# GRIPS-code/pyLBL

Hardware: AMD Instinct MI355X
Metric: line×gridpoint Voigt evals/sec (whole job; per GPU: evals_per_s_per_gpu; spectra/sec: spectra_per_s) (higher is better)
Workload: dtype f64; 1 GPU; BASELINE config 'target': 1 level(s) per GPU, H2O+CO2, grid 1-5000 cm-1 at 0.001 cm-1 (5000000 points), cut_off 25, remove_pedestal=False; levels_total=1, atmosphere=surface, output=gas, parallelism=levels sharded

## Files before the change

### pylbl_amd/abi.py

```python
from ctypes import CDLL, POINTER, Structure, byref, c_char_p, c_double, c_int32, c_int64, \
                   c_void_p
import os
from pathlib import Path

import numpy as np

from .errors import EngineError

LIBRARY_PATH = Path(__file__).resolve().parent / "liblbl_amd.so"

LBL_OK = 0
TABLE_OPEN_FAILED, TABLE_NO_ALIAS, TABLE_NO_TIPS, TABLE_NOT_RECTANGULAR, TABLE_NO_ISOTOPOLOGUES, \
    TABLE_NO_TRANSITIONS = 10, 11, 12, 13, 14, 15
RANGE_REFERENCE, RANGE_SKIP = 0, 1
PREP_DEVICE, PREP_HOST = 0, 1
OUT_DEVICE, ASYNC, SCALE_DENSITY, ACCUMULATE, FARFIELD, DEFER_FINISH = 1, 2, 4, 8, 16, 32
RANGE_POLICIES = {"reference": RANGE_REFERENCE, "skip": RANGE_SKIP}
PATH_OPTICAL_DEPTH, PATH_TRANSMITTANCE, PATH_CUMULATIVE, PATH_FROM_LAST, PATH_CONTINUE = \
    0x100, 0x200, 0x400, 0x800, 0x1000
PATH_RADIANCE, PATH_BRIGHTNESS = 0x2000, 0x4000
PATH_FLUX_UP = 0x8000
PATH_JACOBIAN_DEPTH, PATH_JACOBIAN_LOG_DEPTH, PATH_JACOBIAN_TEMPERATURE, \
    PATH_JACOBIAN_BOUNDARY_T, PATH_JACOBIAN_BOUNDARY_E = \
    0x10000, 0x20000, 0x40000, 0x80000, 0x100000
# ... 92 lines not shown
    "lbl_table_read": [c_char_p, c_char_p, POINTER(c_void_p)],
    "lbl_table_shape": [_ptr, _i64p, _i32p, _i32p, _i32p, _i32p, c_char_p, _i32],
    "lbl_table_copy": [_ptr] + [_ptr]*6,
    "lbl_table_free": [_ptr],
    "lbl_molecule_load_sqlite": [_ptr, c_char_p, c_char_p, _i32p],
    "lbl_compat_state": [_i32p, _i32p],
    "lbl_version": [],
    "lbl_wing_batches": [_ptr],
    "lbl_solar_spectrum": [_ptr, _i32, _i64, _i32, _ptr, _ptr, _f64, _f64, _ptr, _i32],
    "lbl_path_solar": _BLOCK + _RUN + [_ptr]*6 + [_i32] + [_ptr]*10 + [_i32],
    "lbl_band_distribution": [_ptr, _ptr, _i64, _i64, _i32, _ptr, _i32, _ptr, _ptr, _i32, _ptr,
                              _ptr, _ptr, _i32, _ptr, _i32],
}
RESULT_TYPES = {"lbl_last_error": c_char_p, "lbl_stream": c_void_p, "lbl_version": c_char_p}
EXPORTED_SYMBOLS = tuple(PROTOTYPES)
TWO_STREAM_PROTOTYPES = {
    "lbl_rayleigh_row": [_ptr, _i32, _i64, _ptr, _ptr, _i32],
    "lbl_path_two_stream": _BLOCK + _RUN + [_ptr]*6 + [_i32] + [_ptr]*18 + [_i32],
}
THERMAL_PROTOTYPES = {
    "lbl_path_thermal_two_stream": _BLOCK + [_i32] + _RUN + [_ptr, _f64, _ptr, _ptr, _ptr, _i32] +
                                   [_ptr]*10 + [_i32],
}
THERMAL_SOURCE_PROTOTYPES = {
    "lbl_path_thermal_two_stream_source": _BLOCK + [_i32] + _RUN + [_ptr, _ptr, _f64, _ptr, _ptr,
                                                                    _ptr, _i32] + [_ptr]*10 +
                                          [_i32],
}
KDIST_PROTOTYPES = {
    "lbl_band_distribution_weighted": [_ptr, _ptr, _i64, _i64, _i32, _ptr, _i32, _ptr, _i32,
                                       _ptr, _ptr, _ptr, _ptr, _i64, _ptr, _ptr, _ptr, _i32,
                                       _ptr, _ptr, _ptr, _ptr, _ptr, _i32, _ptr, _i32],
}
SCATTERER_PROTOTYPES = {
    "lbl_path_two_stream_spectral": _BLOCK + _RUN + [_ptr, _i32, _i32, _ptr, _ptr] + [_ptr]*5 +
                                    [_i32] + [_ptr]*18 + [_i32],
    "lbl_path_thermal_two_stream_spectral": _BLOCK + [_i32] + _RUN + [_ptr, _ptr, _i32, _ptr, _ptr,
                                                                      _f64, _ptr, _ptr, _ptr,
                                                                      _i32] + [_ptr]*10 + [_i32],
}
THERMAL_RADIANCE_PROTOTYPES = {
    "lbl_path_thermal_radiance": _BLOCK + [_i32] + _RUN + [_ptr, _f64] + [_ptr]*6 + [_i32] +
                                 [_ptr]*4 + [_i32],
}

_library = None


def _preload_hip_runtime():
    import importlib.util
    import os
    import sys
    from ctypes import RTLD_GLOBAL
    if "torch" in sys.modules:
        return
    try:
        spec = importlib.util.find_spec("torch")
    except (ImportError, ValueError):
        spec = None
    if spec is None or not spec.submodule_search_locations:
        return
    for location in spec.submodule_search_locations:
        candidate = os.path.join(location, "lib", "libamdhip64.so")
        if os.path.exists(candidate):
            try:
                CDLL(candidate, mode=RTLD_GLOBAL)
            except OSError:
                pass
            return


def library():
    global _library
    if _library is not None:
        return _library
    path = LIBRARY_PATH
    if os.environ.get("PYLBL_AMD_LIBRARY"):
        path = Path(os.environ["PYLBL_AMD_LIBRARY"]).resolve()
        if not path.exists():
            raise EngineError(f"$PYLBL_AMD_LIBRARY names {path}, which does not exist.")
    elif not LIBRARY_PATH.exists():
        try:
            from . import build
            build.build()
        except Exception as error:
            raise EngineError(
                f"{LIBRARY_PATH} is missing and could not be built ({error}); build it with "
                "`python -m pylbl_amd.build` (there is no CPU fallback).")
    _preload_hip_runtime()
    lib = CDLL(str(path))
    for name, arguments in list(PROTOTYPES.items()) + list(TWO_STREAM_PROTOTYPES.items()) + \
            list(THERMAL_PROTOTYPES.items()) + list(THERMAL_SOURCE_PROTOTYPES.items()) + \
            list(KDIST_PROTOTYPES.items()) + list(SCATTERER_PROTOTYPES.items()) + \
            list(THERMAL_RADIANCE_PROTOTYPES.items()):
        function = getattr(lib, name)
        function.argtypes = arguments
        function.restype = RESULT_TYPES.get(name, c_int32)
    _library = lib
    return lib


def read_line_table(path, name):
    from ctypes import create_string_buffer
    lib = library()
    table = c_void_p()
    status = lib.lbl_table_read(os.fsencode(str(path)), str(name).encode(), byref(table))
    if status != LBL_OK:
        return status, lib.lbl_last_error(None).decode(), None
    try:
        n_lines, molecule_id = c_int64(), c_int32()
        rows, num_iso, num_t = c_int32(), c_int32(), c_int32()
        formula = create_string_buffer(256)
        lib.lbl_table_shape(table, byref(n_lines), byref(molecule_id), byref(rows), byref(num_iso),
                            byref(num_t), formula, 256)
        columns = np.empty((7, n_lines.value))
        local_iso_id = np.empty(n_lines.value, dtype=np.int32)
        isoid = np.empty(rows.value, dtype=np.int64)
        mass = np.empty(rows.value)
        tips_temperature = np.empty(num_t.value)
        tips_data = np.empty((num_iso.value, num_t.value))
        lib.lbl_table_copy(table, columns.ctypes.data, local_iso_id.ctypes.data, isoid.ctypes.data,
                           mass.ctypes.data, tips_temperature.ctypes.data, tips_data.ctypes.data)
    finally:
        lib.lbl_table_free(table)
    return LBL_OK, "", {"formula": formula.value.decode(), "molecule_id": molecule_id.value,
                        "columns": columns, "local_iso_id": local_iso_id, "isoid": isoid,
                        "mass": mass, "tips_temperature": tips_temperature,
# ... 2 lines not shown
```

### pylbl_amd/csrc/accumulate.h

```cpp
#pragma once

#include <hip/hip_runtime.h>

#include "line_prep.h"
#include "voigt_profile.h"

namespace lbl {

struct Tiling
{
    int aligned;
    int per_cell;
    int length;
    int n_tiles;
};

__host__ __device__ inline void tile_bounds(const Tiling & t, int tile, int n_per_v, int n,
                                            long long & i0, long long & i1)
{
    if (t.aligned)
    {
        const int cell = tile/t.per_cell;
        const int sub = tile - cell*t.per_cell;
        i0 = (long long)cell*n_per_v + (long long)sub*t.length;
// ... 19 lines not shown
{
    const double v_lo = (double)v0 + (double)i0*dv;
    const double v_hi = (double)v0 + (double)i1*dv;
    return 0.5*(v_lo + v_hi);
}

#ifndef LBL_WING_GROUP
#define LBL_WING_GROUP 8
#endif
#ifndef LBL_FAR_TERMS
#define LBL_FAR_TERMS 21
#define LBL_FAR_RATIO 4.
#endif
constexpr int kFarTerms = LBL_FAR_TERMS;
constexpr double kFarRatio = LBL_FAR_RATIO;

struct alignas(16) WorkItem
{
    int tile;
    int part, parts;
    int slot;
};

struct AccumulateArgs
{
    const LineWing * wing;
    const LineCore * core;
    const TileSchedule * schedule;
    const LevelScalars * levels;
    const WorkItem * items;
    const double * far_series;
    const int * wing_bounds;
    int wing_batches;
    double * partial;
    long long partial_slots;
    double * k;
    long long level_stride;
    long long n_lines;
    Tiling tiling;
    int n_tiles;
    int n;
    int v0, n_per_v;
    double dv;
    double v0_real;
    int scale_density;
    int accumulate;
    int inner_everywhere;
#ifdef LBL_ABLATE
    int ablate;
#endif
};

#ifdef LBL_ABLATE
#define LBL_ABLATED(a, bits) (((a).ablate & (bits)) != 0)
#else
#define LBL_ABLATED(a, bits) false
#endif

}

#include "accumulate_lines.h"

namespace lbl {

__device__ __forceinline__ void share_of(int j0, int j1, int part, int parts, float inverse,
                                         int unit_shift, int & begin, int & end)
// ... 29 lines not shown
#pragma unroll
    for (int p = 0; p < P; ++p)
    {
        const double step = (first_index + (double)(p*64))*a.dv;
        v[p] = a.v0_real + step;
        acc[p] = 0.;
    }

    const int piece = item.part*4 + wave, pieces = item.parts*4;
    GeneralList g;
    int fa0, fa1, fb0, fb1, e;
    const bool clipped_in_groups = !a.inner_everywhere && !LBL_ABLATED(a, 64);
    const float inverse = 1.f/(float)pieces;
    share_of(sc.lo, sc.a1, piece, pieces, inverse, clipped_in_groups ? 3 : 0, g.begin[0], e);
    g.count[0] = e - g.begin[0];
    share_of(sc.c1, sc.c2, piece, pieces, inverse, 0, g.begin[1], e);
    g.count[1] = e - g.begin[1];
    share_of(sc.a2, sc.hi, piece, pieces, inverse, clipped_in_groups ? 3 : 0, g.begin[2], e);
    g.count[2] = e - g.begin[2];
    share_of(sc.f1, sc.c1, piece, pieces, inverse, 2, fa0, fa1);
    share_of(sc.c2, sc.f2, piece, pieces, inverse, 2, fb0, fb1);
    g.begin[3] = fa0 + ((fa1 - fa0) & ~3);
    g.count[3] = (fa1 - fa0) & 3;
    g.begin[4] = fb0 + ((fb1 - fb0) & ~3);
    g.count[4] = (fb1 - fb0) & 3;
    if (LBL_ABLATED(a, 4)) { g.count[0] = 0; g.count[2] = 0; }
    if (LBL_ABLATED(a, 8)) { g.count[3] = 0; g.count[4] = 0; }
    if (LBL_ABLATED(a, 16)) { g.count[1] = 0; }
    if (!LBL_ABLATED(a, 2))
    {
        int batches = 1;
        if (P == 4)
        {
            const int * __restrict__ wb = a.wing_bounds + level*kWingBounds;
            const int bound[kWingBounds] = {wb[0], wb[1], wb[2], wb[3]};
            batches = __builtin_amdgcn_readfirstlane(min(wing_batches(bound), a.wing_batches));
        }
        fast_ranges<P>(wing, fa0, fa1, fb0, fb1, batches, v, acc);
    }
    bool slab_in_use = false;
    if (!LBL_ABLATED(a, 1))
    {
        GeneralList walk = g;
        if (clipped_in_groups)
        {
            clipped_ranges<P>(wing, core, g.begin[0], g.count[0], g.begin[2], g.count[2], i0, i1,
                              lane, v, acc);
            walk.count[0] = walk.count[2] = 0;
        }
        general_ranges<P>(wing, core, walk, i0, i1, lane, v, acc);
        if (!LBL_ABLATED(a, 32) && a.levels[level].inner_possible != 0.)
        {
            GeneralList inner = g;
            if (!a.inner_everywhere)
            {
                inner.count[0] = inner.count[2] = inner.count[3] = inner.count[4] = 0;
            }
            slab_in_use = inner_ranges(wing, core, inner, inner_stage[wave], i0, i1, a.v0,
                                       a.n_per_v, a.dv, lane, slab, P);
        }
    }

#pragma unroll
    for (int p = 0; p < P; ++p)
    {
        partial[wave][p][lane] = slab_in_use ? partial[wave][p][lane] + acc[p] : acc[p];
    }
    __syncthreads();

    const bool add_series = a.far_series != nullptr && item.part == 0;
    const double * __restrict__ series = a.far_series +
        ((long long)level*a.n_tiles + tile)*kFarTerms;
    const double u0 = tile_centre(a.v0, a.dv, first_point, last_point);
    auto series_at = [&](double vv) {
        const double u = vv - u0;
        double value = series[kFarTerms - 1];
#pragma unroll
        for (int k = kFarTerms - 2; k >= 0; --k)
        {
            value = __builtin_fma(value, u, series[k]);
        }
        return value;
    };
// ... 113 lines not shown
```

### pylbl_amd/csrc/accumulate_lines.h

```cpp
#pragma once

namespace lbl {

template <int P>
__device__ __forceinline__ void fast_ranges(const LineWing * __restrict__ wing,
                                            int a0, int a1, int b0, int b1, int batches,
                                            const double (&v)[P], double (&acc)[P])
{
    const int qa = (a1 - a0) >> 2;
    const int quads = qa + ((b1 - b0) >> 2);
    int q = 0;
#if LBL_WING_GROUP == 8
    auto eight = [&](int at, WingTerm (&l)[8]) {
        const int ja = at < qa ? a0 + 4*at : b0 + 4*(at - qa);
        const int jb = (at + 1) < qa ? a0 + 4*(at + 1) : b0 + 4*(at + 1 - qa);
#pragma unroll
        for (int i = 0; i < 4; ++i)
        {
            const LineWing wa = wing[ja + i], wb = wing[jb + i];
            l[i] = WingTerm{wa.centre, wa.g2, wa.bl};
            l[4 + i] = WingTerm{wb.centre, wb.g2, wb.bl};
        }
    };
    if (P == 4 && batches > 1)
// ... 385 lines not shown
        return sum + chain_row(l, c, d);
    }
    double num, den;
    row_quotient(l, q, kind, d, num, den);
    return __builtin_fma(num, rcp_newton(den), sum);
}

template <int P>
__device__ __forceinline__ void core_pair(const LineWing & la, const LineWing & lb,
                                          const LineCore * __restrict__ pair,
                                          unsigned rows_a, unsigned rows_b,
                                          const double (&v)[P], double (&acc)[P])
{
    const RegionOne qa = region_one_of(pair), qb = region_one_of(pair + 1);
#pragma unroll
    for (int p = 0; p < P; ++p)
    {
        const double da = v[p] - la.centre, db = v[p] - lb.centre;
        if (__builtin_expect(((rows_a | rows_b) & (0x100u << p)) == 0, 1))
        {
            double na, ta, nb, tb;
            row_quotient(la, qa, rows_a >> p, da, na, ta);
            row_quotient(lb, qb, rows_b >> p, db, nb, tb);
            acc[p] = __builtin_fma(__builtin_fma(na, tb, nb*ta), rcp_newton(ta*tb), acc[p]);
        }
        else
        {
            acc[p] = single_row(la, qa, pair, rows_a >> p, da, acc[p]);
            acc[p] = single_row(lb, qb, pair + 1, rows_b >> p, db, acc[p]);
        }
    }
}

template <int P>
__device__ __forceinline__ void core_lines(const LineWing * __restrict__ wing,
                                           const LineCore * __restrict__ core,
                                           int begin, int count, int i0, int lane,
                                           const double (&v)[P], double (&acc)[P])
{
    for (int base = 0; base < count; base += 64)
    {
        const int n = min(64, count - base);
        const LineCore * __restrict__ mine = core + begin + base + min(lane, n - 1);
        const unsigned all_region_one = rows_inside(mine->mid_first, mine->mid_last, i0, P) &
                                        ~rows_meeting(mine->hole_first, mine->hole_last, i0, P);
        const unsigned near_core = rows_meeting(mine->core_first, mine->core_last, i0, P);
        const unsigned packed = all_region_one | ((near_core & ~all_region_one) << 8);
        for (int k = 0; k < n; k += 2)
        {
            const int j = begin + base + k;
            const LineWing la = wing[j], lb = wing[j + 1];
            core_pair<P>(la, lb, core + j,
                         (unsigned)__builtin_amdgcn_readlane((int)packed, k),
                         (unsigned)__builtin_amdgcn_readlane((int)packed, k + 1), v, acc);
        }
    }
}

template <int P>
__device__ __forceinline__ void general_ranges(const LineWing * __restrict__ wing,
                                               const LineCore * __restrict__ core,
                                               const GeneralList & g, int i0, int i1, int lane,
                                               const double (&v)[P], double (&acc)[P])
{
    core_lines<P>(wing, core, g.begin[1], g.count[1] & ~1, i0, lane, v, acc);
    GeneralList rest = g;
    rest.begin[1] = g.begin[1] + (g.count[1] & ~1);
    rest.count[1] = g.count[1] & 1;
    const int total = rest.count[0] + rest.count[1] + rest.count[2] + rest.count[3] + rest.count[4];
    for (int k = 0; k < total; ++k)
    {
        const int j = general_index(rest, k);
        const LineWing l = wing[j];
        const LineCore c = core[j];
        general_line<P>(l, &c, i0, i1, lane, v, acc);
    }
}

template <int P>
__device__ __forceinline__ void clipped_ranges(const LineWing * __restrict__ wing,
                                               const LineCore * __restrict__ core,
                                               int begin0, int count0, int begin1, int count1,
                                               int i0, int i1, int lane,
                                               const double (&v)[P], double (&acc)[P])
{
    const int total = count0 + count1;
    int k = 0;
    while (k < total)
    {
        const int j = k < count0 ? begin0 + k : begin1 + (k - count0);
        const bool room = k < count0 ? k + 8 <= count0 : k + 8 <= total;
        if (room)
        {
            const LineWing * __restrict__ mine = wing + j + (lane & 7);
            const int my_first = mine->first, my_last = mine->last;
            WingTerm l[8];
#pragma unroll
            for (int i = 0; i < 8; ++i)
// ... 61 lines not shown
```

### pylbl_amd/csrc/compute_stages.inc

```
namespace {

struct CallShape
{
    Molecule * m = nullptr;
    GridSpec g;
    long long n_long = 0;
    long long stride = 0;
    RangeRule rule;
    Tiling tiling;
    int farfield = 0;
    int points = 0;
};

int shape_of(lbl_engine * engine, const ComputeRequest & rq, CallShape & s)
{
    s.m = find_molecule(engine, rq.molecule);
    if (s.m == nullptr) return fail(engine, LBL_BAD_ARGUMENT, "unknown molecule handle.");
    if (rq.n_levels < 1 || rq.temperature == nullptr || rq.pressure == nullptr ||
        rq.vmr == nullptr)
    {
        return fail(engine, LBL_BAD_ARGUMENT, "need at least one level with T, P and x.");
    }
    if (rq.n_per_v < 1 || rq.vn <= rq.v0 || rq.cut_off < 0)
    {
// ... 158 lines not shown
    const Molecule::Plan & plan;
    bool streamed;
    int pieces;
    bool with_pedestal;
    long long out_bytes;
    long long chunk;
};

void reserve_for_call(const LinesCall & c)
{
    const ComputeRequest & rq = c.rq;
    const CallShape & s = c.shape;
    const CallTraits & t = c.traits;
    Lane & lane = c.lane;
    const long long n_lines = s.m->n_lines, n_tiles = s.tiling.n_tiles, chunk = c.chunk;
    lane.level_feed.refill((size_t)chunk);
    lane.levels.reserve((size_t)chunk);
    lane.wing.reserve((size_t)(chunk*std::max(n_lines, 1ll)));
    lane.core.reserve((size_t)(chunk*std::max(n_lines, 1ll)));
    lane.schedule.reserve((size_t)(chunk*n_tiles));
    if (t.want_k && !t.out_device) lane.staging.reserve((size_t)(chunk*s.n_long));
    if (c.with_pedestal && t.out_device && t.add_into_block)
    {
        lane.raw.reserve((size_t)(chunk*s.n_long));
    }
    if (t.want_k && s.farfield)
    {
        lane.far_series.reserve((size_t)(chunk*n_tiles*kFarTerms));
    }
    if (t.want_k)
    {
        lane.partial.reserve((size_t)std::max(1ll, chunk*c.plan.partial_slots*64*s.points));
    }
    lane.wing_bounds.reserve((size_t)(chunk*kWingBounds));
    if (rq.evals != nullptr)
    {
        lane.evals.reserve(1);
        HIP_TRY(hipMemsetAsync(lane.evals.data, 0, sizeof(unsigned long long), c.stream));
    }
    if (rq.derived != nullptr) lane.derived.reserve((size_t)(std::max(n_lines, 1ll)*8));
}

void launch_far_series(lbl_engine * engine, Lane & lane, const CallShape & s, int count,
                       hipStream_t stream)
{
    const GridSpec & g = s.g;
    const int n_tiles = s.tiling.n_tiles;
    const int n_groups = (n_tiles + kFarGroup - 1)/kFarGroup;
    const long long n_lines = s.m->n_lines;
    engine->timed(kTimeSchedule, stream, [&] {
        dim3 far_grid((unsigned)(((n_groups + 7)/8)*8), (unsigned)count);
        hipLaunchKernelGGL(farfield_series_kernel, far_grid, dim3(256), 0, stream, lane.wing.data,
                           lane.schedule.data, s.m->d_column[0].data, lane.levels.data, n_lines,
                           s.tiling, n_groups, g.v0, g.n_per_v, g.n, g.dv, lane.far_series.data);
        HIP_TRY(hipGetLastError());
    }, 1);
}

void bound_inner_regions(const Molecule & m, const RangeRule & rule, LevelScalars & lv)
{
    lv.inner_possible = 1.;
    const double foreign = lv.p_atm - lv.p_partial;
    if (foreign >= 0. && lv.p_partial >= 0. && m.min_gamma_air >= 0. &&
        m.min_gamma_self >= 0. && m.n_lines > 0)
    {
        double widest = 0.;
        for (int slot = 0; slot < kMassSlots; ++slot)
// ... 42 lines not shown

int inner_points_everywhere(const LevelScalars * levels, int count, const ComputeRequest & rq,
                            const CallShape & s)
{
    double reach = 0.;
    for (int l = 0; l < count; ++l)
    {
        const LevelScalars & lv = levels[l];
        const double kk = lv.core_reach;
        reach = std::max(reach, kk < 0.5 ? kk*(rq.vn + 1.)/(1. - kk) + 2.*lv.shift_max : 1.e9);
    }
    const double tile_width = (double)s.tiling.length*s.g.dv;
    return (rq.cut_off - 1. <= reach + tile_width + 1.) ? 1 : 0;
}

struct HostPrep
{
    std::vector<LineWing> wing;
    std::vector<LineCore> core;
    std::vector<double> derived;
    std::vector<int> wing_bounds;
};

void prepare_on_host(lbl_engine * engine, Lane & lane, const ComputeRequest & rq,
                     const CallShape & s, int count, hipStream_t stream, HostPrep & hp)
{
    const Molecule & m = *s.m;
    const long long n_lines = m.n_lines;
    if (n_lines > 0)
    {
        hp.wing.resize((size_t)(count*n_lines));
        hp.core.resize((size_t)(count*n_lines));
        if (rq.derived != nullptr) hp.derived.assign((size_t)(n_lines*8), 0.);
        hp.wing_bounds.assign((size_t)(count*kWingBounds), kWingBoundsFill);
        unsigned long long total = 0;
        for (int l = 0; l < count; ++l)
        {
            for (long long j = 0; j < n_lines; ++j)
            {
                const bool ok = m.iso_slot[j] >= 0 &&
                                line_accepted(s.rule, m.column[0][j], m.order[j]);
                double * d = (rq.derived != nullptr && l == 0) ? hp.derived.data() + j*8
                                                               : nullptr;
                LineWing & w = hp.wing[(size_t)(l*n_lines + j)];
                const int status = prepare_line(
                    lane.level_feed.block[l], s.g, m.column[0][j], m.column[1][j], m.column[2][j],
                    m.column[3][j], m.column[4][j], m.column[5][j], m.column[6][j],
                    std::max(m.iso_slot[j], 0), ok, w, hp.core[(size_t)(l*n_lines + j)], d);
                if (status == 1 && w.last >= w.first) total += w.last - w.first + 1;
                int bound[kWingBounds];
                wing_line_bounds(s.g, m.column[0][j], status, w,
                                 hp.core[(size_t)(l*n_lines + j)], bound);
                for (int b = 0; b < kWingBounds; ++b)
                {
                    int & least = hp.wing_bounds[(size_t)(l*kWingBounds + b)];
                    least = std::min(least, bound[b]);
                }
            }
        }
        engine->timed(kTimePrepare, stream, [&] {
            HIP_TRY(hipMemcpyAsync(lane.wing.data, hp.wing.data(),
                                   hp.wing.size()*sizeof(LineWing), hipMemcpyHostToDevice,
                                   stream));
            HIP_TRY(hipMemcpyAsync(lane.core.data, hp.core.data(),
                                   hp.core.size()*sizeof(LineCore), hipMemcpyHostToDevice,
                                   stream));
            HIP_TRY(hipMemcpyAsync(lane.wing_bounds.data, hp.wing_bounds.data(),
                                   hp.wing_bounds.size()*sizeof(int), hipMemcpyHostToDevice,
                                   stream));
        });
        HIP_TRY(hipStreamSynchronize(stream));
        if (rq.evals != nullptr) *rq.evals += (int64_t)total;
    }
    if (rq.k != nullptr)
    {
        engine->timed(kTimeSchedule, stream, [&] {
            dim3 grid((unsigned)((8ll*s.tiling.n_tiles + 255)/256), (unsigned)count);
            hipLaunchKernelGGL(schedule_kernel, grid, dim3(256), 0, stream, m.view(),
                               lane.levels.data, s.g, s.tiling, s.farfield, lane.schedule.data);
            HIP_TRY(hipGetLastError());
        });
    }
}

void launch_prologue(const LinesCall & c, int count, HostPrep & hp)
{
    lbl_engine * engine = c.engine;
    const ComputeRequest & rq = c.rq;
    const CallShape & s = c.shape;
    Lane & lane = c.lane;
    hipStream_t stream = c.stream;
    if (engine->prep == LBL_PREP_HOST)
    {
        prepare_on_host(engine, lane, rq, s, count, stream, hp);
        return;
    }
    const bool inline_levels = levels_inline(engine, count);
    InlineLevels packed;
    if (inline_levels)
    {
        std::memcpy(packed.level, lane.level_feed.block, count*sizeof(LevelScalars));
    }
    const int prepare_blocks = (int)((s.m->n_lines + 255)/256);
    const int schedule_blocks = c.traits.want_k ? (int)((8ll*s.tiling.n_tiles + 255)/256) : 0;
    HIP_TRY(hipMemsetAsync(lane.wing_bounds.data, 0x7f, (size_t)count*kWingBounds*sizeof(int),
                           stream));
    engine->timed(kTimePrepare, stream, [&] {
        dim3 grid((unsigned)std::max(prepare_blocks + schedule_blocks, 1), (unsigned)count);
        hipLaunchKernelGGL(prologue_kernel, grid, dim3(256), 0, stream, s.m->view(),
                           lane.levels.data, packed, inline_levels ? 1 : 0, s.g, s.rule, s.tiling,
                           s.farfield, prepare_blocks, lane.wing.data, lane.core.data,
                           lane.schedule.data,
                           rq.derived != nullptr ? lane.derived.data : nullptr,
                           rq.evals != nullptr ? lane.evals.data : nullptr,
                           lane.wing_bounds.data);
        HIP_TRY(hipGetLastError());
    });
}

Lane::Pass pass_of(const LinesCall & c, long long base, int count)
{
    const CallTraits & t = c.traits;
    Lane::Pass p;
    p.base = base;
    p.count = count;
    p.target = t.out_device ? c.rq.k + base*c.shape.stride : c.lane.staging.data;
    p.target_stride = t.out_device ? c.shape.stride : c.shape.n_long;
    p.sums = p.target;
    p.sums_stride = p.target_stride;
    if (c.with_pedestal && t.out_device && t.add_into_block)
    {
        p.sums = c.lane.raw.data;
        p.sums_stride = c.shape.n_long;
    }
    p.ped_stream = c.engine->overlap_pedestal ? c.lane.side : c.stream;
    p.finish_stream = c.with_pedestal ? p.ped_stream : c.stream;
    return p;
}
// ... 4 lines not shown
    Lane & lane = c.lane;
    if (engine->overlap_pedestal)
    {
        lane.prepared.record(c.stream);
        HIP_TRY(hipStreamWaitEvent(lane.side, lane.prepared, 0));
    }
    engine->timed(kTimePedestal, p.ped_stream, [&] {
        pedestal_find_runs(lane.pedestal, p.ped_stream, c.shape.m->view(), lane.wing.data,
                           c.shape.g, p.count, c.rq.vn - c.rq.v0, engine->scan_chain != 0,
                           engine->poison_workspace != 0);
    }, 0);
    if (engine->overlap_pedestal)
    {
        lane.runs_found.record(lane.side);
    }
}

AccumulateArgs accumulate_args(const LinesCall & c, const Lane::Pass & p)
{
    const ComputeRequest & rq = c.rq;
    const CallShape & s = c.shape;
    const GridSpec & g = s.g;
    const Lane & lane = c.lane;
    const bool add_into = c.traits.out_device && c.traits.add_into_block;
    AccumulateArgs args;
    args.wing = lane.wing.data;
    args.core = lane.core.data;
    args.schedule = lane.schedule.data;
    args.levels = lane.levels.data;
    args.items = c.plan.items.data;
    args.far_series = s.farfield ? lane.far_series.data : nullptr;
    args.wing_bounds = lane.wing_bounds.data;
    args.wing_batches = c.engine->wing_batches;
    args.partial = lane.partial.data;
    args.partial_slots = c.plan.partial_slots;
    args.level_stride = p.sums_stride;
    args.k = p.sums;
    args.n_lines = s.m->n_lines;
    args.tiling = s.tiling;
    args.n_tiles = s.tiling.n_tiles;
    args.n = g.n;
    args.v0 = g.v0;
    args.n_per_v = g.n_per_v;
    args.dv = g.dv;
    args.v0_real = (double)g.v0;
    args.scale_density = (!c.with_pedestal && (rq.flags & LBL_SCALE_DENSITY)) ? 1 : 0;
    args.accumulate = (!c.with_pedestal && add_into) ? 1 : 0;
    args.inner_everywhere = inner_points_everywhere(lane.level_feed.block, p.count, rq, s);
#ifdef LBL_ABLATE
    args.ablate = c.engine->ablate;
#endif
    return args;
}

void launch_piece(const LinesCall & c, const Lane::Pass & p, const AccumulateArgs & args,
                  int piece)
{
    const Molecule::Plan & plan = c.plan;
    hipStream_t stream = c.stream;
    const int points = c.shape.points, count = p.count;
    const int item0 = plan.item_begin[piece], item1 = plan.item_begin[piece + 1];
    const int split0 = plan.split_begin[piece], split1 = plan.split_begin[piece + 1];
    c.engine->timed(kTimeAccumulate, stream, [&] {
        if (item1 > item0)
        {
            AccumulateArgs mine = args;
// ... 165 lines not shown
```

### pylbl_amd/csrc/engine.hip

```cpp
#include <hip/hip_runtime.h>

#include <algorithm>
#include <cmath>
#include <cstdio>
#include <cstring>
#include <functional>
#include <limits>
#include <memory>
#include <mutex>
#include <numeric>
#include <string>
#include <vector>

#include "../../include/lbl_amd.h"
#include "../../include/lbl_amd_twostream.h"
#include "../../include/lbl_amd_thermal.h"
#include "../../include/lbl_amd_thermal_source.h"
#include "../../include/lbl_amd_kdist.h"
#include "../../include/lbl_amd_scatterer.h"
#include "../../include/lbl_amd_thermal_radiance.h"
#include "accumulate.h"
#include "band_sort.h"
#include "band_sort_pairs.h"
#include "continuum.h"
#include "xsec.h"
#include "farfield.h"
#include "flux.h"
#include "instrument.h"
#include "jacobian.h"
#include "line_prep.h"
#include "path.h"
#include "pedestal.h"
#include "radiance.h"
#include "solar.h"
#include "surface.h"
#include "tile_schedule.h"
#include "twostream.h"
#include "twostream_thermal.h"
#include "thermal_radiance.h"

#include "engine_core.h"
#include "lanes_plans.inc"
#include "compute_stages.inc"
#include "compute_call.inc"

#include "delivery.inc"
#include "slot_entry.inc"

extern "C" {

const char * lbl_version(void)
{
    return "pylbl_amd 0.1 (gfx950)";
}

int lbl_wing_batches(const int32_t * bounds)
{
    if (bounds == nullptr) return 1;
    const int bound[kWingBounds] = {bounds[0], bounds[1], bounds[2], bounds[3]};
    return wing_batches(bound);
}

int lbl_engine_create(int device, lbl_engine ** engine)
{
    if (engine == nullptr) return fail(nullptr, LBL_BAD_ARGUMENT, "engine is NULL.");
    *engine = nullptr;
    int count = 0;
    if (hipGetDeviceCount(&count) != hipSuccess || count <= 0)
    {
        return fail(nullptr, LBL_NO_DEVICE,
                    "no HIP device visible: this engine has no CPU fallback.");
    }
    if (device < 0 || device >= count)
    {
        return fail(nullptr, LBL_NO_DEVICE, "device index out of range.");
    }
    try
    {
        HIP_TRY(hipSetDevice(device));
        std::unique_ptr<lbl_engine> e(new lbl_engine());
        e->device = device;
        for (int i = 0; i < kAllLanes; ++i) e->lanes[i].create(i == kSlotLane);
        e->stream = e->lanes[0].main;
        e->copy_stream.create();
        calibrate_delivery_lanes(e.get());
        e->copies_handed_over.create();
        e->taken_over.create();
        *engine = e.release();
    }
    catch (const HipFailure & f)
    {
        return fail(nullptr, LBL_NO_DEVICE, f.message);
    }
// ... 291 lines not shown
        }
        else if (key == "skip_delivery_lanes" && (value == 0 || value == 1))
        {
            engine->skip_delivery_lanes = (int)value;
        }
        else if (key == "overlap_plain" && (value == 0 || value == 1))
        {
            engine->overlap_plain = (int)value;
        }
        else if (key == "small_points" && value >= 0)
        {
            engine->small_points = value;
        }
        else if (key == "lanes" && (value == 0 || (value >= 2 && value <= kLanes)))
        {
            engine->lanes_in_use = (int)value;
        }
        else if (key == "farfield" && (value == 0 || value == 1))
        {
            engine->farfield = (int)value;
        }
        else if (key == "overlap_pedestal" && (value == 0 || value == 1))
        {
            engine->overlap_pedestal = (int)value;
        }
        else if (key == "aligned_tiles" && (value == 0 || value == 1))
        {
            engine->aligned_tiles = (int)value;
        }
        else if (key == "wing_batches" && (value == 1 || value == 2 || value == 4 || value == 8))
        {
            engine->wing_batches = std::min((int)value, kWingBatchesMax);
        }
#ifdef LBL_ABLATE
        else if (key == "ablate" && value >= 0 && value <= 127)
        {
            engine->ablate = (int)value;
        }
#endif
        else if (key == "workspace_bytes" && value >= (1 << 20))
        {
            engine->workspace_bytes = value;
        }
        else
        {
            return fail(engine, LBL_BAD_ARGUMENT, "unknown option or value: " + key);
        }
        return LBL_OK;
    });
}

int lbl_timing(lbl_engine * engine, double ms[8], int64_t launches[8], int32_t reset)
{
    return entry(engine, [&] {
        HIP_TRY(hipSetDevice(engine->device));
        engine->drain_lanes();
        engine->drain_spans();
        for (int i = 0; i < kTimeKinds; ++i)
        {
            if (ms != nullptr) ms[i] = engine->time_ms[i];
            if (launches != nullptr) launches[i] = engine->launches[i];
            if (reset)
            {
                engine->time_ms[i] = 0.;
                engine->launches[i] = 0;
                engine->busy_ms[i] = 0.;
// ... 39 lines not shown
```

### pylbl_amd/csrc/engine_core.h

```cpp
#pragma once

#include "hip_owners.h"

namespace {

using namespace lbl;

thread_local std::string g_create_error;
thread_local std::string g_thread_error;
thread_local const void * g_thread_error_engine = nullptr;

struct Molecule
{
    long long n_lines = 0;
    std::vector<double> nu_row;
    bool ascending = true;
    std::vector<int> order;
    std::vector<double> column[7];
    std::vector<int> iso_slot;
    double mass[kMassSlots];
    unsigned used_slots = 0;
    struct BadRow { int row; double nu; int local_iso_id; };
    std::vector<BadRow> bad_rows;
    double max_abs_delta = 0.;
// ... 208 lines not shown
    DeviceBuffer<double> tables;
    DeviceBuffer<double> partial;
    PinnedFeed<double> staged;
};

}

struct lbl_engine
{
    std::recursive_mutex mutex;
    int device = 0;
    hipStream_t stream = nullptr;
    bool delivers_badly[kLanes] = {};
    Event copies_handed_over, taken_over;
    Stream copy_stream;
    std::string error;
    std::vector<std::unique_ptr<Molecule>> molecules;
    std::vector<std::unique_ptr<ContinuumSet>> continua;
    std::vector<std::unique_ptr<SpectralGrid>> grids;
    std::vector<std::unique_ptr<XsecData>> xsecs;
    std::vector<std::unique_ptr<ContinuumGroup>> groups;
    std::vector<std::unique_ptr<Instrument>> instruments;
    Lane lanes[kAllLanes];
    unsigned next_lane = 0;
    PathWorkspace path;

    int prep = LBL_PREP_DEVICE;
    int points_per_lane = 0;
    int timing = 0;
    long long workspace_bytes = 4ll << 30;
    int ablate = 0;
    int aligned_tiles = 0;
    int wing_batches = kWingBatchesMax;
    int overlap_pedestal = 1;
    int farfield = 0;
    int scan_chain = 1;
    int relax_launches = 0;
    int poison_workspace = 0;
    int lanes_in_use = 0;
    long long small_points = 1ll << 20;
    int overlap_plain = 1;
    int skip_delivery_lanes = 1;

    struct Span { Event begin, end; int kind, counts; };
    std::vector<Span> spans;
    std::vector<Event> event_pool;
    double time_ms[kTimeKinds] = {};
    double busy_ms[kTimeKinds] = {};
    double busy_reach[kTimeKinds] = {};
    Event epoch;
    long long launches[kTimeKinds] = {};

    Event take_event()
    {
        Event e(true);
        if (!event_pool.empty())
        {
            e = std::move(event_pool.back());
            event_pool.pop_back();
        }
        e.create();
        return e;
    }

    ~lbl_engine()
    {
// ... 247 lines not shown
```

### pylbl_amd/csrc/line_prep.h

```cpp
#pragma once

#include <hip/hip_runtime.h>
#include <math.h>
#include <stdint.h>

namespace lbl {

constexpr int kMassSlots = 32;
constexpr double kPi = 3.14159265358979323846;

struct LevelScalars
{
    double temperature;
    double p_atm;
    double p_partial;
    double tfact;
    double t_minus_ref;
    double t_times_ref;
    double shift_max;
    double core_reach;
    double density;
    double inner_possible;
    double doppler[kMassSlots];
    double q_ratio[kMassSlots];
// ... 35 lines not shown
__host__ __device__ inline void mark_empty(LineWing & w, LineCore & c)
{
    w.centre = 0.; w.g2 = 1.; w.bl = 0.; w.first = kEmptyFirst; w.last = kEmptyLast;
    c.A = 1.; c.B = 0.; c.A2 = 1.;
    c.repwid = 1.; c.y = 100.; c.amp = 0.; c.xlim0 = 0.; c.xlim1 = 0.;
    c.core_first = kEmptyFirst; c.core_last = kEmptyLast;
    c.mid_first = kEmptyFirst; c.mid_last = kEmptyLast;
    c.hole_first = kEmptyFirst; c.hole_last = kEmptyLast;
    for (int i = 0; i < 10; ++i) c.pad[i] = 0;
}

__host__ __device__ inline void inner_index_range(double centre, double repwid, double xlim1,
                                                  int v0, int n_per_v, int & first, int & last)
{
    const double near = (xlim1/repwid)*(1. + 1.e-9);
    double lo = floor((centre - near - (double)v0)*n_per_v) - 1.;
    double hi = floor((centre + near - (double)v0)*n_per_v) + 2.;
    if (lo < -1.e9) lo = -1.e9;
    if (hi > 1.e9) hi = 1.e9;
    if (hi < -1.e9) hi = -1.e9;
    if (lo > 1.e9) lo = 1.e9;
    first = (int)lo;
    last = (int)hi;
}

enum WingBound
{
    kWingTLow,
    kWingTHighNeg,
    kWingBLow,
    kWingBHighNeg,
    kWingBounds
};
constexpr int kWingBoundsFill = 0x7f7f7f7f;
#ifndef LBL_WING_BATCHES
#define LBL_WING_BATCHES 8
#endif
constexpr int kWingBatchesMax = LBL_WING_BATCHES;

__host__ __device__ inline int wing_exponent_low(double x)
{
    return (x > 0. && x < 1.e300) ? ilogb(x) : -4096;
}

__host__ __device__ inline int wing_exponent_high(double x)
{
    return (x > 0. && x < 1.e300) ? ilogb(x) + 1 : 4096;
}

__host__ __device__ inline void wing_line_bounds(const GridSpec & g, double nu, int status,
                                                 const LineWing & w, const LineCore & c,
                                                 int (&bound)[kWingBounds])
{
    bound[kWingTLow] = bound[kWingTHighNeg] = kWingBoundsFill;
    bound[kWingBLow] = bound[kWingBHighNeg] = kWingBoundsFill;
    if (status == 1 && w.last >= w.first)
    {
        const double reach = c.xlim0 > 0. ? (c.xlim0/c.repwid)*(1. - 1.e-6) : 0.;
        const double far = (double)g.cut_off + 1.;
        bound[kWingTLow] = wing_exponent_low(reach*reach + w.g2);
        bound[kWingTHighNeg] = -wing_exponent_high(far*far + w.g2);
        const double b = fabs(w.bl);
        if (b != 0.)
        {
            bound[kWingBLow] = wing_exponent_low(b);
            bound[kWingBHighNeg] = -wing_exponent_high(b);
        }
    }
    else if (status == -1 && nu >= (double)(g.v0 - g.cut_off - 1) &&
             nu < (double)(g.vn + g.cut_off))
    {
        const double v = fmax(fabs((double)g.v0), fabs((double)g.vn));
        bound[kWingTHighNeg] = -wing_exponent_high(v*v + 1.);
    }
}

__host__ __device__ inline int wing_batches(const int (&bound)[kWingBounds])
{
    const long long t_lo = bound[kWingTLow], t_hi = -(long long)bound[kWingTHighNeg];
    long long b_lo = bound[kWingBLow], b_hi = -(long long)bound[kWingBHighNeg];
    if (t_lo == kWingBoundsFill || -t_hi == kWingBoundsFill)
    {
        return 1;
    }
    if (b_lo == kWingBoundsFill)
    {
        b_lo = b_hi = 0;
    }
    if (t_lo < -2000 || t_hi > 2000 || b_lo < -2000 || b_hi > 2000)
    {
        return 1;
    }
    for (int k = kWingBatchesMax; k > 1; k >>= 1)
    {
        const long long n = 8*k;
        const long long lowest = (t_lo < 0 ? n*t_lo : (n - 1)*t_lo) + (b_lo < 0 ? b_lo : 0);
        const long long highest = (t_hi > 0 ? n*t_hi : (n - 1)*t_hi) + (b_hi > 0 ? b_hi : 0) + 6;
        if (lowest >= -1000 && highest <= 1000 && n*t_lo >= -1000 && n*t_hi <= 1000)
        {
            return k;
        }
    }
    return 1;
}

__host__ __device__ inline int prepare_line(const LevelScalars & lv, const GridSpec & g,
                                            double nu, double sw, double gamma_air,
                                            double gamma_self, double n_air, double elower,
                                            double delta_air, int iso_slot, bool accepted,
                                            LineWing & w, LineCore & c, double * derived)
{
    const double vlight = 2.99792458e8;
    const double c2 = 1.4387752;
    const double rsqrpi = 1./sqrt(kPi);
    const double sqrln2 = sqrt(log(2.));
    mark_empty(w, c);
    if (derived != nullptr)
    {
        for (int i = 0; i < 8; ++i) derived[i] = 0.;
        derived[6] = -1.;
    }
    if (!accepted)
    {
        return -1;
    }
    const double centre = nu + lv.p_atm*delta_air;
    const double gamma = (gamma_air*(lv.p_atm - lv.p_partial) + gamma_self*lv.p_partial)*
                         pow(lv.tfact, n_air);
    const double alpha = (nu/vlight)*lv.doppler[iso_slot];
    const double sb = exp(elower*c2*lv.t_minus_ref/lv.t_times_ref);
    const double gg = exp((-c2*nu)/lv.temperature);
// ... 77 lines not shown
```

### pylbl_amd/csrc/tile_schedule.h

```cpp
#pragma once

#include <hip/hip_runtime.h>

#include "accumulate.h"
#include "line_prep.h"

namespace lbl {

struct LineTableView
{
    const double * nu;
    const double * sw;
    const double * gamma_air;
    const double * gamma_self;
    const double * n_air;
    const double * elower;
    const double * delta_air;
    const int * iso_slot;
    const int * row;
    const int * sorted_of_row;
    long long n_lines;
    const int * cell_first;
    double cell_base, cell_scale;
    int cell_entries;
// ... 125 lines not shown
}

__global__ __launch_bounds__(256) void schedule_kernel(const LineTableView table,
                                                       const LevelScalars * __restrict__ levels,
                                                       const GridSpec g, const Tiling tiling,
                                                       const int farfield,
                                                       TileSchedule * __restrict__ schedule)
{
    const int thread = blockIdx.x*blockDim.x + threadIdx.x;
    const int tile = thread >> 3;
    const int level = blockIdx.y;
    const bool active = tile < tiling.n_tiles;
    schedule_tile(table, levels[level], g, tiling, farfield, tile, thread & 7, active,
                  schedule + (long long)level*tiling.n_tiles + (active ? tile : 0));
}

constexpr int kInlineLevels = 4;
struct InlineLevels
{
    LevelScalars level[kInlineLevels];
};

__device__ __forceinline__ void prepare_block(const LineTableView & t, const LevelScalars & lv,
                                              const GridSpec & g, const RangeRule & rule,
                                              int block, int level,
                                              LineWing * __restrict__ wing,
                                              LineCore * __restrict__ core,
                                              double * __restrict__ derived,
                                              unsigned long long * __restrict__ evals,
                                              int * __restrict__ wing_bounds)
{
    const long long j = (long long)block*blockDim.x + threadIdx.x;
    unsigned long long count = 0;
    int bound[kWingBounds] = {kWingBoundsFill, kWingBoundsFill, kWingBoundsFill, kWingBoundsFill};
    if (j < t.n_lines)
    {
        LineWing w;
        LineCore c;
        const double nu = t.nu[j];
        const int slot = t.iso_slot[j];
        const bool ok = slot >= 0 && line_accepted(rule, nu, t.row[j]);
        double * d = derived != nullptr ? derived + ((long long)level*t.n_lines + j)*8 : nullptr;
        const int status = prepare_line(lv, g, nu, t.sw[j], t.gamma_air[j],
                                        t.gamma_self[j], t.n_air[j], t.elower[j],
                                        t.delta_air[j], max(slot, 0), ok, w, c, d);
        wing[(long long)level*t.n_lines + j] = w;
        core[(long long)level*t.n_lines + j] = c;
        if (status == 1 && w.last >= w.first)
        {
            count = (unsigned long long)(w.last - w.first + 1);
        }
        wing_line_bounds(g, nu, status, w, c, bound);
    }
    {
        __shared__ int block_bound[4][kWingBounds];
#pragma unroll
        for (int b = 0; b < kWingBounds; ++b)
        {
            for (int offset = 32; offset > 0; offset >>= 1)
            {
                bound[b] = min(bound[b], __shfl_down(bound[b], offset, 64));
            }
        }
        const int wave = threadIdx.x >> 6;
        if ((threadIdx.x & 63) == 0)
        {
#pragma unroll
            for (int b = 0; b < kWingBounds; ++b) block_bound[wave][b] = bound[b];
        }
        __syncthreads();
        if (threadIdx.x < kWingBounds)
        {
            const int b = threadIdx.x;
            const int least = min(min(block_bound[0][b], block_bound[1][b]),
                                  min(block_bound[2][b], block_bound[3][b]));
            if (least != kWingBoundsFill)
            {
                atomicMin(wing_bounds + (long long)level*kWingBounds + b, least);
            }
        }
    }
    if (evals != nullptr)
    {
        for (int offset = 32; offset > 0; offset >>= 1)
        {
            count += __shfl_down(count, offset, 64);
        }
        if ((threadIdx.x & 63) == 0 && count != 0)
        {
            atomicAdd(evals, count);
        }
    }
}

__global__ __launch_bounds__(256) void prologue_kernel(const LineTableView t,
                                                       LevelScalars * __restrict__ levels,
                                                       const InlineLevels inline_levels,
                                                       const int use_inline,
                                                       const GridSpec g, const RangeRule rule,
                                                       const Tiling tiling, const int farfield,
                                                       const int prepare_blocks,
                                                       LineWing * __restrict__ wing,
                                                       LineCore * __restrict__ core,
                                                       TileSchedule * __restrict__ schedule,
                                                       double * __restrict__ derived,
                                                       unsigned long long * __restrict__ evals,
                                                       int * __restrict__ wing_bounds)
{
    const int level = blockIdx.y;
    const LevelScalars & lv = use_inline ? inline_levels.level[level] : levels[level];
    if (use_inline && blockIdx.x == 0)
// ... 20 lines not shown
```

Before: 6592 billion evals/s.

## Batch core-line rational sums into running fractions to defer reciprocals

```diff
diff --git a/include/lbl_amd_core.h b/include/lbl_amd_core.h
--- /dev/null
+++ b/include/lbl_amd_core.h
@@ -0,0 +1,15 @@
+#ifndef LBL_AMD_CORE_H_
+#define LBL_AMD_CORE_H_
+
+#include "lbl_amd.h"
+
+#ifdef __cplusplus
+extern "C" {
+#endif
+
+int lbl_core_groups(const int32_t *bounds);
+
+#ifdef __cplusplus
+}
+#endif
+#endif
diff --git a/pylbl_amd/abi.py b/pylbl_amd/abi.py
--- a/pylbl_amd/abi.py
+++ b/pylbl_amd/abi.py
@@ -148,6 +148,9 @@
                                        _ptr, _ptr, _ptr, _ptr, _i64, _ptr, _ptr, _ptr, _i32,
                                        _ptr, _ptr, _ptr, _ptr, _ptr, _i32, _ptr, _i32],
 }
+CORE_PROTOTYPES = {
+    "lbl_core_groups": [_ptr],
+}
 SCATTERER_PROTOTYPES = {
     "lbl_path_two_stream_spectral": _BLOCK + _RUN + [_ptr, _i32, _i32, _ptr, _ptr] + [_ptr]*5 +
                                     [_i32] + [_ptr]*18 + [_i32],
@@ -208,7 +211,7 @@
     for name, arguments in list(PROTOTYPES.items()) + list(TWO_STREAM_PROTOTYPES.items()) + \
             list(THERMAL_PROTOTYPES.items()) + list(THERMAL_SOURCE_PROTOTYPES.items()) + \
             list(KDIST_PROTOTYPES.items()) + list(SCATTERER_PROTOTYPES.items()) + \
-            list(THERMAL_RADIANCE_PROTOTYPES.items()):
+            list(THERMAL_RADIANCE_PROTOTYPES.items()) + list(CORE_PROTOTYPES.items()):
         function = getattr(lib, name)
         function.argtypes = arguments
         function.restype = RESULT_TYPES.get(name, c_int32)
diff --git a/pylbl_amd/csrc/accumulate.h b/pylbl_amd/csrc/accumulate.h
--- a/pylbl_amd/csrc/accumulate.h
+++ b/pylbl_amd/csrc/accumulate.h
@@ -75,6 +75,7 @@
     const double * far_series;
     const int * wing_bounds;
     int wing_batches;
+    int core_groups;
     double * partial;
     long long partial_slots;
     double * k;
@@ -170,7 +171,7 @@
         int batches = 1;
         if (P == 4)
         {
-            const int * __restrict__ wb = a.wing_bounds + level*kWingBounds;
+            const int * __restrict__ wb = a.wing_bounds + level*kLevelBounds;
             const int bound[kWingBounds] = {wb[0], wb[1], wb[2], wb[3]};
             batches = __builtin_amdgcn_readfirstlane(min(wing_batches(bound), a.wing_batches));
         }
@@ -186,7 +187,14 @@
                               lane, v, acc);
             walk.count[0] = walk.count[2] = 0;
         }
-        general_ranges<P>(wing, core, walk, i0, i1, lane, v, acc);
+        int groups = 1;
+        if (P <= 4)
+        {
+            const int * __restrict__ cb = a.wing_bounds + level*kLevelBounds + kWingBounds;
+            const int bound[kCoreBounds] = {cb[0], cb[1], cb[2], cb[3]};
+            groups = __builtin_amdgcn_readfirstlane(min(core_groups(bound), a.core_groups));
+        }
+        general_ranges<P>(wing, core, walk, groups, i0, i1, lane, v, acc);
         if (!LBL_ABLATED(a, 32) && a.levels[level].inner_possible != 0.)
         {
             GeneralList inner = g;
diff --git a/pylbl_amd/csrc/accumulate_lines.h b/pylbl_amd/csrc/accumulate_lines.h
--- a/pylbl_amd/csrc/accumulate_lines.h
+++ b/pylbl_amd/csrc/accumulate_lines.h
@@ -441,10 +441,65 @@
     }
 }
 
+template <int P, bool kOpen>
+__device__ __forceinline__ void core_pair_running(const LineWing & la, const LineWing & lb,
+                                                  const LineCore * __restrict__ pair,
+                                                  unsigned rows_a, unsigned rows_b,
+                                                  const double (&v)[P], double (&acc)[P],
+                                                  double (&num)[P], double (&den)[P])
+{
+    const RegionOne qa = region_one_of(pair), qb = region_one_of(pair + 1);
+#pragma unroll
+    for (int p = 0; p < P; ++p)
+    {
+        const double da = v[p] - la.centre, db = v[p] - lb.centre;
+        double n, t;
+        if (__builtin_expect(((rows_a | rows_b) & (0x100u << p)) == 0, 1))
+        {
+            double na, ta, nb, tb;
+            row_quotient(la, qa, rows_a >> p, da, na, ta);
+            row_quotient(lb, qb, rows_b >> p, db, nb, tb);
+            n = __builtin_fma(na, tb, nb*ta);
+            t = ta*tb;
+        }
+        else if ((rows_a & rows_b) & (0x100u << p))
+        {
+            acc[p] += chain_row(la, pair, da);
+            acc[p] += chain_row(lb, pair + 1, db);
+            if (kOpen)
+            {
+                num[p] = 0.;
+                den[p] = 1.;
+            }
+            continue;
+        }
+        else if (rows_a & (0x100u << p))
+        {
+            acc[p] += chain_row(la, pair, da);
+            row_quotient(lb, qb, rows_b >> p, db, n, t);
+        }
+        else
+        {
+            row_quotient(la, qa, rows_a >> p, da, n, t);
+            acc[p] += chain_row(lb, pair + 1, db);
+        }
+        if (kOpen)
+        {
+            num[p] = n;
+            den[p] = t;
+        }
+        else
+        {
+            num[p] = __builtin_fma(n, den[p], num[p]*t);
+            den[p] = den[p]*t;
+        }
+    }
+}
+
 template <int P>
 __device__ __forceinline__ void core_lines(const LineWing * __restrict__ wing,
                                            const LineCore * __restrict__ core,
-                                           int begin, int count, int i0, int lane,
+                                           int begin, int count, int groups, int i0, int lane,
                                            const double (&v)[P], double (&acc)[P])
 {
     for (int base = 0; base < count; base += 64)
@@ -455,6 +510,35 @@
                                         ~rows_meeting(mine->hole_first, mine->hole_last, i0, P);
         const unsigned near_core = rows_meeting(mine->core_first, mine->core_last, i0, P);
         const unsigned packed = all_region_one | ((near_core & ~all_region_one) << 8);
+        if (P <= 4 && groups > 1)
+        {
+            for (int k = 0; k < n; )
+            {
+                const int stop = min(k + 2*groups, n);
+                double num[P], den[P];
+                {
+                    const int j = begin + base + k;
+                    const LineWing la = wing[j], lb = wing[j + 1];
+                    core_pair_running<P, true>(
+                        la, lb, core + j, (unsigned)__builtin_amdgcn_readlane((int)packed, k),
+                        (unsigned)__builtin_amdgcn_readlane((int)packed, k + 1), v, acc, num, den);
+                }
+                for (k += 2; k < stop; k += 2)
+                {
+                    const int j = begin + base + k;
+                    const LineWing la = wing[j], lb = wing[j + 1];
+                    core_pair_running<P, false>(
+                        la, lb, core + j, (unsigned)__builtin_amdgcn_readlane((int)packed, k),
+                        (unsigned)__builtin_amdgcn_readlane((int)packed, k + 1), v, acc, num, den);
+                }
+#pragma unroll
+                for (int p = 0; p < P; ++p)
+                {
+                    acc[p] = __builtin_fma(num[p], rcp_newton(den[p]), acc[p]);
+                }
+            }
+            continue;
+        }
         for (int k = 0; k < n; k += 2)
         {
             const int j = begin + base + k;
@@ -469,10 +553,11 @@
 template <int P>
 __device__ __forceinline__ void general_ranges(const LineWing * __restrict__ wing,
                                                const LineCore * __restrict__ core,
-                                               const GeneralList & g, int i0, int i1, int lane,
+                                               const GeneralList & g, int groups, int i0,
+                                               int i1, int lane,
                                                const double (&v)[P], double (&acc)[P])
 {
-    core_lines<P>(wing, core, g.begin[1], g.count[1] & ~1, i0, lane, v, acc);
+    core_lines<P>(wing, core, g.begin[1], g.count[1] & ~1, groups, i0, lane, v, acc);
     GeneralList rest = g;
     rest.begin[1] = g.begin[1] + (g.count[1] & ~1);
     rest.count[1] = g.count[1] & 1;
diff --git a/pylbl_amd/csrc/compute_stages.inc b/pylbl_amd/csrc/compute_stages.inc
--- a/pylbl_amd/csrc/compute_stages.inc
+++ b/pylbl_amd/csrc/compute_stages.inc
@@ -214,7 +214,7 @@
     {
         lane.partial.reserve((size_t)std::max(1ll, chunk*c.plan.partial_slots*64*s.points));
     }
-    lane.wing_bounds.reserve((size_t)(chunk*kWingBounds));
+    lane.wing_bounds.reserve((size_t)(chunk*kLevelBounds));
     if (rq.evals != nullptr)
     {
         lane.evals.reserve(1);
@@ -323,7 +323,7 @@
         hp.wing.resize((size_t)(count*n_lines));
         hp.core.resize((size_t)(count*n_lines));
         if (rq.derived != nullptr) hp.derived.assign((size_t)(n_lines*8), 0.);
-        hp.wing_bounds.assign((size_t)(count*kWingBounds), kWingBoundsFill);
+        hp.wing_bounds.assign((size_t)(count*kLevelBounds), kWingBoundsFill);
         unsigned long long total = 0;
         for (int l = 0; l < count; ++l)
         {
@@ -339,12 +339,12 @@
                     m.column[3][j], m.column[4][j], m.column[5][j], m.column[6][j],
                     std::max(m.iso_slot[j], 0), ok, w, hp.core[(size_t)(l*n_lines + j)], d);
                 if (status == 1 && w.last >= w.first) total += w.last - w.first + 1;
-                int bound[kWingBounds];
+                int bound[kLevelBounds];
                 wing_line_bounds(s.g, m.column[0][j], status, w,
                                  hp.core[(size_t)(l*n_lines + j)], bound);
-                for (int b = 0; b < kWingBounds; ++b)
+                for (int b = 0; b < kLevelBounds; ++b)
                 {
-                    int & least = hp.wing_bounds[(size_t)(l*kWingBounds + b)];
+                    int & least = hp.wing_bounds[(size_t)(l*kLevelBounds + b)];
                     least = std::min(least, bound[b]);
                 }
             }
@@ -394,7 +394,7 @@
     }
     const int prepare_blocks = (int)((s.m->n_lines + 255)/256);
     const int schedule_blocks = c.traits.want_k ? (int)((8ll*s.tiling.n_tiles + 255)/256) : 0;
-    HIP_TRY(hipMemsetAsync(lane.wing_bounds.data, 0x7f, (size_t)count*kWingBounds*sizeof(int),
+    HIP_TRY(hipMemsetAsync(lane.wing_bounds.data, 0x7f, (size_t)count*kLevelBounds*sizeof(int),
                            stream));
     engine->timed(kTimePrepare, stream, [&] {
         dim3 grid((unsigned)std::max(prepare_blocks + schedule_blocks, 1), (unsigned)count);
@@ -465,6 +465,7 @@
     args.far_series = s.farfield ? lane.far_series.data : nullptr;
     args.wing_bounds = lane.wing_bounds.data;
     args.wing_batches = c.engine->wing_batches;
+    args.core_groups = c.engine->core_groups;
     args.partial = lane.partial.data;
     args.partial_slots = c.plan.partial_slots;
     args.level_stride = p.sums_stride;
diff --git a/pylbl_amd/csrc/engine.hip b/pylbl_amd/csrc/engine.hip
--- a/pylbl_amd/csrc/engine.hip
+++ b/pylbl_amd/csrc/engine.hip
@@ -17,6 +17,7 @@
 #include "../../include/lbl_amd_thermal.h"
 #include "../../include/lbl_amd_thermal_source.h"
 #include "../../include/lbl_amd_kdist.h"
+#include "../../include/lbl_amd_core.h"
 #include "../../include/lbl_amd_scatterer.h"
 #include "../../include/lbl_amd_thermal_radiance.h"
 #include "accumulate.h"
@@ -59,6 +60,13 @@
     if (bounds == nullptr) return 1;
     const int bound[kWingBounds] = {bounds[0], bounds[1], bounds[2], bounds[3]};
     return wing_batches(bound);
+}
+
+int lbl_core_groups(const int32_t * bounds)
+{
+    if (bounds == nullptr) return 1;
+    const int bound[kCoreBounds] = {bounds[0], bounds[1], bounds[2], bounds[3]};
+    return core_groups(bound);
 }
 
 int lbl_engine_create(int device, lbl_engine ** engine)
@@ -416,6 +424,10 @@
         {
             engine->wing_batches = std::min((int)value, kWingBatchesMax);
         }
+        else if (key == "core_groups" && (value == 1 || value == 2 || value == 4 || value == 8))
+        {
+            engine->core_groups = std::min((int)value, kCoreGroupsMax);
+        }
 #ifdef LBL_ABLATE
         else if (key == "ablate" && value >= 0 && value <= 127)
         {
diff --git a/pylbl_amd/csrc/engine_core.h b/pylbl_amd/csrc/engine_core.h
--- a/pylbl_amd/csrc/engine_core.h
+++ b/pylbl_amd/csrc/engine_core.h
@@ -264,6 +264,7 @@
     int ablate = 0;
     int aligned_tiles = 0;
     int wing_batches = kWingBatchesMax;
+    int core_groups = kCoreGroupsMax;
     int overlap_pedestal = 1;
     int farfield = 0;
     int scan_chain = 1;
diff --git a/pylbl_amd/csrc/line_prep.h b/pylbl_amd/csrc/line_prep.h
--- a/pylbl_amd/csrc/line_prep.h
+++ b/pylbl_amd/csrc/line_prep.h
@@ -91,11 +91,24 @@
     kWingBHighNeg,
     kWingBounds
 };
+enum CoreBound
+{
+    kCoreTLow = kWingBounds,
+    kCoreTHighNeg,
+    kCoreNLow,
+    kCoreNHighNeg,
+    kLevelBounds
+};
+constexpr int kCoreBounds = kLevelBounds - kWingBounds;
 constexpr int kWingBoundsFill = 0x7f7f7f7f;
 #ifndef LBL_WING_BATCHES
 #define LBL_WING_BATCHES 8
 #endif
 constexpr int kWingBatchesMax = LBL_WING_BATCHES;
+#ifndef LBL_CORE_GROUPS
+#define LBL_CORE_GROUPS 8
+#endif
+constexpr int kCoreGroupsMax = LBL_CORE_GROUPS;
 
 __host__ __device__ inline int wing_exponent_low(double x)
 {
@@ -109,10 +122,9 @@
 
 __host__ __device__ inline void wing_line_bounds(const GridSpec & g, double nu, int status,
                                                  const LineWing & w, const LineCore & c,
-                                                 int (&bound)[kWingBounds])
-{
-    bound[kWingTLow] = bound[kWingTHighNeg] = kWingBoundsFill;
-    bound[kWingBLow] = bound[kWingBHighNeg] = kWingBoundsFill;
+                                                 int (&bound)[kLevelBounds])
+{
+    for (int b = 0; b < kLevelBounds; ++b) bound[b] = kWingBoundsFill;
     if (status == 1 && w.last >= w.first)
     {
         const double reach = c.xlim0 > 0. ? (c.xlim0/c.repwid)*(1. - 1.e-6) : 0.;
@@ -125,12 +137,34 @@
             bound[kWingBLow] = wing_exponent_low(b);
             bound[kWingBHighNeg] = -wing_exponent_high(b);
         }
+        int t_lo = bound[kWingTLow], t_hi = -bound[kWingTHighNeg];
+        double n_lo = b, n_hi = b;
+        if (c.xlim0 > 0.)
+        {
+            const double edge = fmin((c.xlim0/c.repwid)*(1. + 1.e-6), far);
+            const double Dmax = edge*edge;
+            const double least = c.B >= 0. ? c.A2 : (w.g2 + w.g2)/(c.repwid*c.repwid);
+            const int one_lo = wing_exponent_low(least);
+            const int one_hi = wing_exponent_high(c.A2 + Dmax*(fabs(c.B) + Dmax));
+            t_lo = one_lo < t_lo ? one_lo : t_lo;
+            t_hi = one_hi > t_hi ? one_hi : t_hi;
+            n_lo = fmin(n_lo, b*c.A);
+            n_hi = fmax(n_hi, b*(c.A + Dmax));
+        }
+        bound[kCoreTLow] = t_lo;
+        bound[kCoreTHighNeg] = -t_hi;
+        if (b != 0.)
+        {
+            bound[kCoreNLow] = wing_exponent_low(n_lo);
+            bound[kCoreNHighNeg] = -wing_exponent_high(n_hi);
+        }
     }
     else if (status == -1 && nu >= (double)(g.v0 - g.cut_off - 1) &&
              nu < (double)(g.vn + g.cut_off))
     {
         const double v = fmax(fabs((double)g.v0), fabs((double)g.vn));
         bound[kWingTHighNeg] = -wing_exponent_high(v*v + 1.);
+        bound[kCoreTHighNeg] = bound[kWingTHighNeg];
     }
 }
 
@@ -156,6 +190,39 @@
         const long long lowest = (t_lo < 0 ? n*t_lo : (n - 1)*t_lo) + (b_lo < 0 ? b_lo : 0);
         const long long highest = (t_hi > 0 ? n*t_hi : (n - 1)*t_hi) + (b_hi > 0 ? b_hi : 0) + 6;
         if (lowest >= -1000 && highest <= 1000 && n*t_lo >= -1000 && n*t_hi <= 1000)
+        {
+            return k;
+        }
+    }
+    return 1;
+}
+
+__host__ __device__ inline int core_groups(const int (&bound)[kCoreBounds])
+{
+    const long long t_lo = bound[kCoreTLow - kWingBounds];
+    const long long t_hi = -(long long)bound[kCoreTHighNeg - kWingBounds];
+    long long n_lo = bound[kCoreNLow - kWingBounds];
+    long long n_hi = -(long long)bound[kCoreNHighNeg - kWingBounds];
+    if (t_lo == kWingBoundsFill || -t_hi == kWingBoundsFill)
+    {
+        return 1;
+    }
+    if (n_lo == kWingBoundsFill)
+    {
+        n_lo = n_hi = 0;
+    }
+    if (t_lo < -2000 || t_hi > 2000 || n_lo < -2000 || n_hi > 2000)
+    {
+        return 1;
+    }
+    for (int k = kCoreGroupsMax; k > 1; k >>= 1)
+    {
+        const long long m = 2*k;
+        const long long t_least = t_lo < 0 ? m*t_lo : t_lo;
+        const long long t_most = t_hi > 0 ? m*t_hi : t_hi;
+        const long long n_least = n_lo + (t_lo < 0 ? (m - 1)*t_lo : 0);
+        const long long n_most = n_hi + (t_hi > 0 ? (m - 1)*t_hi : 0) + 4;
+        if (t_least >= -1000 && t_most <= 1000 && n_least >= -1000 && n_most <= 1000)
         {
             return k;
         }
diff --git a/pylbl_amd/csrc/tile_schedule.h b/pylbl_amd/csrc/tile_schedule.h
--- a/pylbl_amd/csrc/tile_schedule.h
+++ b/pylbl_amd/csrc/tile_schedule.h
@@ -181,7 +181,8 @@
 {
     const long long j = (long long)block*blockDim.x + threadIdx.x;
     unsigned long long count = 0;
-    int bound[kWingBounds] = {kWingBoundsFill, kWingBoundsFill, kWingBoundsFill, kWingBoundsFill};
+    int bound[kLevelBounds];
+    for (int b = 0; b < kLevelBounds; ++b) bound[b] = kWingBoundsFill;
     if (j < t.n_lines)
     {
         LineWing w;
@@ -202,9 +203,9 @@
         wing_line_bounds(g, nu, status, w, c, bound);
     }
     {
-        __shared__ int block_bound[4][kWingBounds];
+        __shared__ int block_bound[4][kLevelBounds];
 #pragma unroll
-        for (int b = 0; b < kWingBounds; ++b)
+        for (int b = 0; b < kLevelBounds; ++b)
         {
             for (int offset = 32; offset > 0; offset >>= 1)
             {
@@ -215,17 +216,17 @@
         if ((threadIdx.x & 63) == 0)
         {
 #pragma unroll
-            for (int b = 0; b < kWingBounds; ++b) block_bound[wave][b] = bound[b];
+            for (int b = 0; b < kLevelBounds; ++b) block_bound[wave][b] = bound[b];
         }
         __syncthreads();
-        if (threadIdx.x < kWingBounds)
+        if (threadIdx.x < kLevelBounds)
         {
             const int b = threadIdx.x;
             const int least = min(min(block_bound[0][b], block_bound[1][b]),
                                   min(block_bound[2][b], block_bound[3][b]));
             if (least != kWingBoundsFill)
             {
-                atomicMin(wing_bounds + (long long)level*kWingBounds + b, least);
+                atomicMin(wing_bounds + (long long)level*kLevelBounds + b, least);
             }
         }
     }
```

New measurement: 6590 billion evals/s, median of 3. No clear change (-0.0%).
